# AIflowerQ/InvPref_KDD_2022

Measured on AMD Instinct MI355X. Metric: training interactions/sec, Yahoo-implicit InvPref, higher is better.
Workload: dtype f32; 1 GPU; yahoo_r3_implicit_shaped; users=15400, items=1000, envs=4, factor_num=64, scaling=strong, interactions_total=250154, global_batch=8192, interactions_per_gpu=250154, batch_per_gpu=8192, estep_every_steps=155, parallelism=single GPU

## Files before the change

invpref_kdd_2022_amd/csrc/step_alt.hpp:

```cpp

#ifdef ALT_STAMPS
#define ASTAMP(i) STAMP(i)
#else
#define ASTAMP(i) do { } while (0)
#endif

struct AltArgs {
    float *own_p[2];
    float *own_m[2], *own_v[2];
    const float *oth_p[2];
    float *Ev, *W, *b;
    float *mEv, *mW, *mb, *vEv, *vW, *vb;
    int E, D;
    const int4 *desc;
    const int4 *pend;
    const int4 *list;
    const int *push_slot;
    const int4 *stream;
    int rounds_per_task, rows_per_stream_task, n_cls;
    int cls[8][4];
    const int64_t *envs;
    const float *weights;
    StepScalars k;
    float r2_prev, r1_prev;
    uint32_t flags;
    int mode;
    AdamScalars ad_cur, ad_prev;
    int gen;
    int *sched_state;
    int sched_slot;
    const SchedRow *sched_table;
    int sched_n;
    const float *pend_rows;
    float *push_rows;
    const float *slabs_prev;
    int n_partials_prev;
    float *slabs;
    int *fold_flags;
    unsigned long long *pub;
    float l2, l1;
    double inv_B_prev, inv_BD2_prev;
    float *losses_prev;
    int fold_blocks, first_task_block;
    int stamps_nodrain;
    unsigned long long *stamps;
};

__device__ __forceinline__ float ld_sc1(const float *p) {
    return __hip_atomic_load(p, __ATOMIC_RELAXED, __HIP_MEMORY_SCOPE_AGENT);
}
__device__ __forceinline__ int ld_sc1(const int *p) {
    return __hip_atomic_load(p, __ATOMIC_RELAXED, __HIP_MEMORY_SCOPE_AGENT);
}
__device__ __forceinline__ void st_sc1(float *p, float v) {
    __hip_atomic_store(p, v, __ATOMIC_RELAXED, __HIP_MEMORY_SCOPE_AGENT);
}
__device__ __forceinline__ void st_sc1(int *p, int v) {
    __hip_atomic_store(p, v, __ATOMIC_RELAXED, __HIP_MEMORY_SCOPE_AGENT);
}

#ifndef ALT_POLL_MAX
#define ALT_POLL_MAX (1 << 17)
#endif
#ifndef ALT_TEST_BAD_TAG
#define ALT_TEST_BAD_TAG 0
#endif
constexpr int kAltStreamDelay = 40;
constexpr int kAltPushSt = 1, kAltSlabSt = 1;
constexpr int kAltPendBatch = 4;

struct AltStage {
    unsigned long long g[9];
    float cw;
};
__device__ __forceinline__ void alt_stage_lanes(const AltArgs &a, int lane, bool (&on)[4], bool &onb) {
    constexpr int DP = 64;
#pragma unroll
    for (int i = 0; i < 4; i++) {
        const int idx = lane + 64 * i, e = idx / DP, d = idx - e * DP;
        on[i] = e < a.E && d < a.D;
    }
    onb = lane < a.E;
}
#define ALT_GRANULE_LOADS                                                                                                     \
    "global_load_dwordx2 %0, %9, %11 sc1\n\t"                                                                              \
    "global_load_dwordx2 %1, %9, %11 offset:512 sc1\n\t"                                                                   \
    "global_load_dwordx2 %2, %9, %11 offset:1024 sc1\n\t"                                                                  \
    "global_load_dwordx2 %3, %9, %11 offset:1536 sc1\n\t"                                                                  \
    "global_load_dwordx2 %4, %9, %11 offset:2048 sc1\n\t"                                                                  \
    "global_load_dwordx2 %5, %9, %11 offset:2560 sc1\n\t"                                                                  \
    "global_load_dwordx2 %6, %9, %11 offset:3072 sc1\n\t"                                                                  \
    "global_load_dwordx2 %7, %9, %11 offset:3584 sc1\n\t"                                                                  \
    "global_load_dwordx2 %8, %10, %11 sc1"
__device__ __forceinline__ void alt_stage_issue(const AltArgs &a, AltStage &x) {
    constexpr int EDP = 4 * 64;
    const int lane = threadIdx.x & 63;
    const unsigned o0 = (unsigned)lane * 8u, ob = (unsigned)(2 * EDP + (lane < a.E ? lane : 0)) * 8u;
    asm volatile(ALT_GRANULE_LOADS
                 : "=&v"(x.g[0]), "=&v"(x.g[1]), "=&v"(x.g[2]), "=&v"(x.g[3]), "=&v"(x.g[4]), "=&v"(x.g[5]), "=&v"(x.g[6]),
                   "=&v"(x.g[7]), "=&v"(x.g[8])
                 : "v"(o0), "v"(ob), "s"(a.pub)
                 : "memory");
    x.cw = ((a.flags & INVPREF_WEIGHTS_BY_ENV) && lane < a.E) ? a.weights[lane] : 1.f;
}
__device__ __forceinline__ void alt_stage_finish(const AltArgs &a, AltStage &x, int gen, float *sEv, float *sW, float *sb, float *scw) {
    constexpr int EMAX = 4, EDP = 4 * 64;
    const int lane = threadIdx.x & 63;
    bool on[4], onb;
    alt_stage_lanes(a, lane, on, onb);
    if (ALT_TEST_BAD_TAG) gen ^= 0x40000000;
    const unsigned o0 = (unsigned)lane * 8u, ob = (unsigned)(2 * EDP + (onb ? lane : 0)) * 8u;
    asm volatile("s_waitcnt vmcnt(0)"
                 : "+v"(x.g[0]), "+v"(x.g[1]), "+v"(x.g[2]), "+v"(x.g[3]), "+v"(x.g[4]), "+v"(x.g[5]), "+v"(x.g[6]), "+v"(x.g[7]),
                   "+v"(x.g[8])
                 :
                 : "memory");
    int polls = 0;
    bool timed_out = false;
    for (;;) {
        bool ok = !onb || (int)(x.g[8] >> 32) == gen;
#pragma unroll
        for (int i = 0; i < 4; i++)
// ... 6 lines not shown
        }
        __builtin_amdgcn_s_sleep(4);
        asm volatile(ALT_GRANULE_LOADS "\n\ts_waitcnt vmcnt(0)"
                     : "=&v"(x.g[0]), "=&v"(x.g[1]), "=&v"(x.g[2]), "=&v"(x.g[3]), "=&v"(x.g[4]), "=&v"(x.g[5]), "=&v"(x.g[6]),
                       "=&v"(x.g[7]), "=&v"(x.g[8])
                     : "v"(o0), "v"(ob), "s"(a.pub)
                     : "memory");
    }
    if (timed_out) {
#pragma unroll
        for (int i = 0; i < 9; i++) x.g[i] = 0x7fc00000ull;
    }
#pragma unroll
    for (int i = 0; i < 4; i++) {
        sEv[lane + 64 * i] = on[i] ? __builtin_bit_cast(float, (unsigned)x.g[i]) : 0.f;
        sW[lane + 64 * i] = on[i] ? __builtin_bit_cast(float, (unsigned)x.g[4 + i]) : 0.f;
    }
    if (lane < EMAX) sb[lane] = onb ? __builtin_bit_cast(float, (unsigned)x.g[8]) : 0.f;
    if (lane < EMAX) scw[lane] = x.cw;
}
__device__ __forceinline__ void alt_stage_plain(const AltArgs &a, float *sEv, float *sW, float *sb, float *scw, bool pure) {
    constexpr int EMAX = 4, DP = 64;
    const int lane = threadIdx.x & 63;
    bool on[4], onb;
    alt_stage_lanes(a, lane, on, onb);
#pragma unroll
    for (int i = 0; i < 4; i++) {
        const int idx = lane + 64 * i, e = idx / DP, d = idx - e * DP;
        const bool o = on[i] && !pure;
        sEv[idx] = o ? a.Ev[e * a.D + d] : 0.f;
        sW[idx] = o ? a.W[e * a.D + d] : 0.f;
    }
    if (lane < EMAX) sb[lane] = (onb && !pure) ? a.b[lane] : 0.f;
    if (lane < EMAX) scw[lane] = ((a.flags & INVPREF_WEIGHTS_BY_ENV) && onb && !pure) ? a.weights[lane] : 1.f;
}

template <int THREADS>
struct AltGeo {
    static constexpr int NG = THREADS / 16, WAVES = THREADS / 64, DP = 64, EMAX = 4;
    static constexpr int SLAB = 2 * EMAX * DP + EMAX + kLossSlots;
    static constexpr int sEv = 0, sW = sEv + EMAX * DP, sb = sW + EMAX * DP;
    static constexpr int scw = sb + EMAX;
    static constexpr int mv = scw + EMAX;
    static constexpr int red = mv + WAVES * 4 * 64 * 4;
    static constexpr int total = red + NG * SLAB;
};

__device__ __forceinline__ void adam4_prev(float4 &p, float4 g, float4 &m, float4 &v, const AdamScalars &ad, float2 prev2) {
    AdamScalars ap = ad;
    ap.step_size = prev2.x; ap.bc2_sqrt = prev2.y;
    adam4(p, g, m, v, ap);
}

template <bool VEC, bool FULL, int MODE, int THREADS>
__device__ __forceinline__ void alt_task(const AltArgs &a, int r0, int slab_index, float *lds,
                                         const AdamScalars &ad_cur, float2 prev2, const StepScalars &k, int gen) {
    constexpr int LG = 16, EMAX = 4, UE = 2;
    using G = AltGeo<THREADS>;
    using L = AltGeo<THREADS>;
    static_assert(EvalLds<16, 4>::total == AltGeo<256>::total, "alt_task: the smallest-instance layout");
    constexpr int NG = G::NG, DP = G::DP;
    float *sEv = lds + L::sEv, *sW = lds + L::sW, *sb = lds + L::sb, *scw = lds + L::scw;
    float4 *mv = reinterpret_cast<float4 *>(lds + L::mv);
    float *red = lds + L::red;
    const int lg = threadIdx.x & (LG - 1), grp = threadIdx.x / LG, wave = threadIdx.x >> 6, lane = threadIdx.x & 63;
    float4 *mv_wave = mv + wave * 4 * 64;
    const bool implicit = a.flags & INVPREF_IMPLICIT;
    const bool rw_rec = a.flags & INVPREF_REWEIGHT_REC, rw_cls = a.flags & INVPREF_REWEIGHT_CLS;
    const bool by_env = a.flags & INVPREF_WEIGHTS_BY_ENV;
    const bool reg_env = a.flags & INVPREF_REG_ENV_EMBED;
    const bool pure = a.flags & INVPREF_PURE_MF;
    const bool dense = (a.flags & INVPREF_DENSE_REG) && !(a.flags & INVPREF_REG_ONLY_EMBED) && !pure;
    constexpr bool has_prev = MODE & 1, has_cur = MODE & 2;
    const int D = a.D;
    float *own0 = a.own_p[0], *own1 = a.own_p[1];
    const float *oth0 = a.oth_p[0], *oth1 = a.oth_p[1];

    ASTAMP(0);
    int4 d = a.desc[(r0 * NG + grp) * 2], d1 = a.desc[(r0 * NG + grp) * 2 + 1];
    int4 pd = make_int4(0, 0, 0, 0);
    if (has_prev) pd = a.pend[r0 * NG + grp];
    ASTAMP(1);
    float accLi = 0.f, accLe = 0.f, accLc = 0.f, accL2 = 0.f, accL1 = 0.f;
    float *slab = a.slabs + (int64_t)slab_index * G::SLAB;
    auto slot_of = [&](int g) {
        constexpr int GW = 64 / LG;
        return lds + L::mv + (g / GW) * (4 * 64 * 4) + (g % GW) * 2 * DP;
    };

    {
        constexpr int nr = 1;
        const int r = r0;
        const int4 dd = d, dd1 = d1;
        const int4 pdd = pd;
        const int row = dd.x, meta = dd.y;
        const bool active = row >= 0, leader = meta & 1;
        const int slices_f = (meta >> 1) & 31, mode = (meta >> 6) & 7;
        const int slices = slices_f ? slices_f : 32;
        const bool rpend = has_prev && (meta < 0);
        const int cnt_i = (meta >> 9) & 0x3fffff;
        const int nsmp = (active && has_cur) ? (mode == 7 ? dd.w - dd.z : mode) : 0;
        if (r == r0 + STAMP_ROUND) ASTAMP(2);
        const int s_lo = dd.z, s_hi1 = max(dd.w - 1, dd.z);
        const int *dwords = reinterpret_cast<const int *>(a.desc + (r * NG + grp) * 2);
        auto sample_at = [&](int sidx) {
            USample sm;
            if (FULL) {
                const int *src = mode == 7 ? reinterpret_cast<const int *>(a.list + min(s_lo + sidx, s_hi1)) : dwords + 2 + 3 * min(sidx, 1);
                sm.oth = src[0]; sm.ps = src[1]; sm.y = __builtin_bit_cast(float, src[2]);
            } else if (mode == 7) {
                const int4 q = a.list[dd.z + sidx];
                sm.oth = q.x; sm.ps = q.y; sm.y = __builtin_bit_cast(float, q.z);
            } else if (sidx == 0) { sm.oth = dd.z; sm.ps = dd.w; sm.y = __builtin_bit_cast(float, dd1.x); }
            else { sm.oth = dd1.y; sm.ps = dd1.z; sm.y = __builtin_bit_cast(float, dd1.w); }
            return sm;
        };
        const int rowc = active ? row : 0;
        float4 oi = row4<VEC, FULL>(own0, rowc, D, lg), oe = f4zero();
        float4 mi = row4<VEC, FULL>(a.own_m[0], rowc, D, lg), vi = row4<VEC, FULL>(a.own_v[0], rowc, D, lg);
        float4 me = f4zero(), ve = f4zero();
        if (!pure) {
            oe = row4<VEC, FULL>(own1, rowc, D, lg);
            me = row4<VEC, FULL>(a.own_m[1], rowc, D, lg); ve = row4<VEC, FULL>(a.own_v[1], rowc, D, lg);
        }
        constexpr int PB = kAltPendBatch;
        static_assert(PB * 2 * 64 * 4 <= 4 * G::SLAB && (4 * G::SLAB) % 4 == 0 && G::red % 4 == 0, "landing block: the wave's four slab rows");
        const int npend = (active && has_prev) ? pdd.y - pdd.x : 0;
        const float *pbase = a.pend_rows + (unsigned)(npend > 0 ? pdd.x : 0) * (unsigned)(2 * DP) + lg * 4;
        float *land = red + wave * 4 * G::SLAB;
        auto pland = [&](int s0) {
#pragma unroll
            for (int j = 0; j < PB; j++) {
                if (s0 + j < npend) {
                    const float *p = pbase + (unsigned)(s0 + j) * (unsigned)(2 * DP);
                    __builtin_amdgcn_global_load_lds((const __attribute__((address_space(1))) void *)p,
                                                     (__attribute__((address_space(3))) void *)(land + (2 * j) * 256), 16, 0, 0);
                    if (!pure)
// ... 144 lines not shown
                        gpi = gpe = f4zero();
#pragma nounroll
                        for (int s = 0; s < slices; s++) {
                            f4add(gpi, *reinterpret_cast<const float4 *>(slot_of(lead + s) + lg * 4));
                            f4add(gpe, *reinterpret_cast<const float4 *>(slot_of(lead + s) + DP + lg * 4));
                        }
                    }
                    __syncthreads();
                }
            }
            const float cp = (float)pdd.z;
            if (cp != 0.f) {
                f4fma(gpi, cp, reg_term(oi, a.r2_prev, a.r1_prev));
                f4fma(gpe, cp, reg_term(oe, a.r2_prev, a.r1_prev));
            }
            adam4_prev(oi, gpi, mi, vi, ad_cur, prev2);
            if (!pure) adam4_prev(oe, gpe, me, ve, ad_cur, prev2);
        }
        if (r == r0 + STAMP_ROUND) ASTAMP(3);
        if (!has_cur) {
            if (active && leader) {
                put4<VEC, 0, FULL>(own0, row, D, lg, oi);
                put4<VEC, 0, FULL>(a.own_m[0], row, D, lg, mi);
                put4<VEC, 0, FULL>(a.own_v[0], row, D, lg, vi);
                if (!pure) {
                    put4<VEC, 0, FULL>(own1, row, D, lg, oe);
                    put4<VEC, 0, FULL>(a.own_m[1], row, D, lg, me);
                    put4<VEC, 0, FULL>(a.own_v[1], row, D, lg, ve);
                }
            }
            return;
        }
        mv_wave[0 * 64 + lane] = mi; mv_wave[1 * 64 + lane] = vi;
        if (!pure) { mv_wave[2 * 64 + lane] = me; mv_wave[3 * 64 + lane] = ve; }
        if (r == r0) {
            {
                constexpr int ZR4 = (2 * EMAX * DP + EMAX) / 4;
                static_assert((2 * EMAX * DP + EMAX) % 4 == 0 && G::SLAB % 4 == 0, "16-byte zeroing");
#pragma unroll
                for (int t = 0; t < (4 * ZR4 + 63) / 64; t++) {
                    const int i = lane + 64 * t;
                    if (i < 4 * ZR4) *reinterpret_cast<float4 *>(land + (i / ZR4) * G::SLAB + (i % ZR4) * 4) = f4zero();
                }
            }
            if (wave == 0) {
                if (has_prev && !pure) alt_stage_issue(a, stg);
                if (has_prev && !pure) alt_stage_finish(a, stg, gen, sEv, sW, sb, scw);
                else alt_stage_plain(a, sEv, sW, sb, scw, pure);
            }
            __syncthreads();
            ASTAMP(4);
        }
        float4 gi = f4zero(), ge = f4zero();
        auto step = [&](const Slot &q, bool has) {
            const int e = q.e;
            if (has) {
                const float wq = by_env ? scw[e] : q.w;
                const float w_rec = rw_rec ? wq : 1.f, w_cls = rw_cls ? wq : 1.f;
                const float4 ev = *reinterpret_cast<const float4 *>(sEv + e * DP + lg * 4);
                Eval<EMAX> o;
                eval_interaction<LG, EMAX>(o, oi, q.qi, oe, q.qa, ev, sW, sb, nullptr, a.E, e, q.sm.y, w_rec * k.invB,
                                           w_cls * k.invB, k, implicit, pure, lg);
                float4 gip;
                gip.x = o.g_p - k.alpha * o.gx.x; gip.y = o.g_p - k.alpha * o.gx.y;
                gip.z = o.g_p - k.alpha * o.gx.z; gip.w = o.g_p - k.alpha * o.gx.w;
                f4add(gi, f4mul(gip, q.qi));
                f4fma(ge, o.g_q, f4mul(q.qa, ev));
                float *cr = a.push_rows + (unsigned)q.cs * (unsigned)(2 * DP) + lg * 4;
                store4<kAltPushSt>(cr, f4mul(gip, oi));
                store4<kAltPushSt>(cr + DP, f4scale(o.g_q, f4mul(oe, ev)));
                float4 oo = f4scale(o.g_q, f4mul(oe, q.qa));
                if (reg_env) f4add(oo, reg_term(ev, 2.f * k.r2, 2.f * k.r1));
                float *mine = red + grp * G::SLAB;
#pragma unroll
                for (int c = 0; c < EMAX; c++) {
                    float4 *wr = reinterpret_cast<float4 *>(mine + EMAX * DP + c * DP + lg * 4);
                    float4 cur = *wr;
                    f4fma(cur, o.gz[c], o.x);
                    *wr = cur;
                }
                if (lg == 0) {
                    float4 *br = reinterpret_cast<float4 *>(mine + 2 * EMAX * DP);
                    float4 cur = *br;
                    cur.x += o.gz[0]; cur.y += o.gz[1]; cur.z += o.gz[2]; cur.w += o.gz[3];
                    *br = cur;
                }
                float4 *erow = reinterpret_cast<float4 *>(mine + e * DP + lg * 4);
                float4 cur = *erow;
                f4add(cur, oo);
                *erow = cur;
                float s2a = 0.f, s2b = 0.f;
                sq_acc(s2a, s2b, q.qi);
                sq_acc(s2a, s2b, q.qa);
                float s2 = s2a + s2b, s1 = abs_acc(abs_acc(0.f, q.qi), q.qa);
                if (reg_env) { s2 += 2.f * f4sq(ev); s1 += 2.f * f4abs(ev); }
                accL2 += s2;
                accL1 += s1;
                if (lg == 0) { accLi += o.li * w_rec; accLe += o.le * w_rec; }
                if (lg == 0) accLc += o.lcls * w_cls;
            }
        };
        for (int s = 0; s < nsmp; s += UE) {
#pragma unroll
            for (int j = 0; j < UE; j++) {
                if (s + j < nsmp) step(sl[j], true);
                if (FULL || s + UE + j < nsmp) gather(sl[j], idn[j]);
                if (FULL || s + 2 * UE + j < nsmp) idn[j] = sample_at(s + 2 * UE + j);
            }
        }
        if (r == r0 + STAMP_ROUND) ASTAMP(5);
        const float cnt = (float)cnt_i;
        if (active && leader) {
            accL2 += cnt * (f4sq(oi) + f4sq(oe));
            accL1 += cnt * (f4abs(oi) + f4abs(oe));
        }
        const bool last = r == r0 + nr - 1;
        if (last) {
            accLi = row16_sum(accLi); accLe = row16_sum(accLe); accLc = row16_sum(accLc);
            accL2 = row16_sum(accL2); accL1 = row16_sum(accL1);
            if (lg == 0) {
                float *ls = red + grp * G::SLAB + 2 * EMAX * DP + EMAX;
                ls[0] = accLi; ls[1] = accLe; ls[2] = accLc; ls[3] = accL2; ls[4] = accL1;
                ls[5] = ls[6] = ls[7] = 0.f;
            }
            if (dense && slab_index == 0 && wave == 0) {
                const float4 w4 = *reinterpret_cast<const float4 *>(sW + lane * 4);
                float w2 = f4sq(w4), w1 = f4abs(w4);
                const float bb = lane < EMAX ? sb[lane] : 0.f;
                float b2 = bb * bb, b1 = fabsf(bb);
                w2 = wave_sum_valu(w2); w1 = wave_sum_valu(w1); b2 = wave_sum_valu(b2); b1 = wave_sum_valu(b1);
                if (lane == 0) {
                    float *ls = red + 2 * EMAX * DP + EMAX;
                    ls[5] = w2 / ((float)a.D * (float)a.E) + b2 / (float)a.E;
                    ls[6] = w1 / ((float)a.D * (float)a.E) + b1 / (float)a.E;
                }
            }
        }
        if (active && leader) {
            mi = mv_wave[0 * 64 + lane]; vi = mv_wave[1 * 64 + lane];
            if (!pure) { me = mv_wave[2 * 64 + lane]; ve = mv_wave[3 * 64 + lane]; }
        }
        asm volatile("" ::: "memory");
        if (slices > 1) {
            float *mine = slot_of(grp);
            *reinterpret_cast<float4 *>(mine + lg * 4) = gi;
            *reinterpret_cast<float4 *>(mine + DP + lg * 4) = ge;
        }
        if (slices > 1 || last) __syncthreads();
        if (last) {
            static_assert(G::SLAB % 4 == 0 && G::SLAB / 4 <= THREADS && NG % 8 == 0, "slab sum: one float4 column set per thread");
            if ((int)threadIdx.x < G::SLAB / 4) {
                const float *col = red + threadIdx.x * 4;
                float4 sum = *reinterpret_cast<const float4 *>(col);
#pragma unroll
                for (int q0 = 0; q0 < NG; q0 += 8) {
                    float4 x[8];
#pragma unroll
                    for (int j = 0; j < 8; j++) x[j] = *reinterpret_cast<const float4 *>(col + (q0 + j) * G::SLAB);
#pragma unroll
                    for (int j = (q0 == 0 ? 1 : 0); j < 8; j++) f4add(sum, x[j]);
                }
                store4<kAltSlabSt>(slab + threadIdx.x * 4, sum);
            }
        }
        if (slices > 1) {
            if (active && leader) {
                if (VEC && slices >= 8) {
                    float4 xi[8], xe[8];
#pragma unroll
                    for (int j = 1; j < 8; j++) {
                        xi[j] = *reinterpret_cast<const float4 *>(slot_of(grp + j) + lg * 4);
                        xe[j] = *reinterpret_cast<const float4 *>(slot_of(grp + j) + DP + lg * 4);
                    }
#pragma unroll
                    for (int j = 1; j < 8; j++) { f4add(gi, xi[j]); f4add(ge, xe[j]); }
#pragma nounroll
                    for (int s = 8; s < slices; s += 8) {
#pragma unroll
                        for (int j = 0; j < 8; j++) {
                            xi[j] = *reinterpret_cast<const float4 *>(slot_of(grp + s + j) + lg * 4);
                            xe[j] = *reinterpret_cast<const float4 *>(slot_of(grp + s + j) + DP + lg * 4);
                        }
#pragma unroll
                        for (int j = 0; j < 8; j++) { f4add(gi, xi[j]); f4add(ge, xe[j]); }
                    }
                } else if (VEC && slices == 4) {
                    float4 xi[4], xe[4];
#pragma unroll
                    for (int j = 1; j < 4; j++) {
                        xi[j] = *reinterpret_cast<const float4 *>(slot_of(grp + j) + lg * 4);
                        xe[j] = *reinterpret_cast<const float4 *>(slot_of(grp + j) + DP + lg * 4);
                    }
#pragma unroll
                    for (int j = 1; j < 4; j++) { f4add(gi, xi[j]); f4add(ge, xe[j]); }
                } else {
#pragma nounroll
                    for (int s = 1; s < slices; s++) {
                        f4add(gi, *reinterpret_cast<const float4 *>(slot_of(grp + s) + lg * 4));
                        f4add(ge, *reinterpret_cast<const float4 *>(slot_of(grp + s) + DP + lg * 4));
                    }
                }
            }
            if (!last) __syncthreads();
        }
        if (r == r0 + STAMP_ROUND) ASTAMP(6);
        if (active && leader) {
            if (cnt != 0.f) {
                f4fma(gi, cnt, reg_term(oi, k.r2, k.r1));
                f4fma(ge, cnt, reg_term(oe, k.r2, k.r1));
            }
            adam4(oi, gi, mi, vi, ad_cur);
            put4<VEC, 0, FULL>(own0, row, D, lg, oi);
            put4<VEC, 0, FULL>(a.own_m[0], row, D, lg, mi);
            put4<VEC, 0, FULL>(a.own_v[0], row, D, lg, vi);
            if (!pure) {
// ... 59 lines not shown
#pragma unroll
        for (int q = 0; q < R; q++) {
            float4 gi = f4zero(), ge = f4zero();
            if (has_prev) {
#pragma unroll
                for (int j = 0; j < H; j++) {
                    f4add(gi, j < npend[q] ? ci[q][j] : f4zero());
                    if (!pure) f4add(ge, j < npend[q] ? ce[q][j] : f4zero());
                }
                const float *pb = a.pend_rows + (unsigned)(npend[q] > 0 ? e[q].y : 0) * (unsigned)(2 * DP) + lg * 4;
                for (int s0 = H; s0 < n_wave; s0 += H) {
                    float4 xi[H], xe[H];
#pragma unroll
                    for (int j = 0; j < H; j++) {
                        const int sj = s0 + j < npend[q] ? s0 + j : (npend[q] > 0 ? npend[q] - 1 : 0);
                        xi[j] = *reinterpret_cast<const float4 *>(pb + (unsigned)sj * (unsigned)(2 * DP));
                        xe[j] = pure ? f4zero() : *reinterpret_cast<const float4 *>(pb + (unsigned)sj * (unsigned)(2 * DP) + DP);
                    }
#pragma unroll
                    for (int j = 0; j < H; j++) {
                        f4add(gi, s0 + j < npend[q] ? xi[j] : f4zero());
                        if (!pure) f4add(ge, s0 + j < npend[q] ? xe[j] : f4zero());
                    }
                }
                const float cp = (float)e[q].w;
                if (cp != 0.f) {
                    f4fma(gi, cp, reg_term(p[2 * q], a.r2_prev, a.r1_prev));
                    f4fma(ge, cp, reg_term(p[2 * q + 1], a.r2_prev, a.r1_prev));
                }
                adam4_prev(p[2 * q], gi, m[2 * q], v[2 * q], ad_cur, prev2);
                if (!pure) adam4_prev(p[2 * q + 1], ge, m[2 * q + 1], v[2 * q + 1], ad_cur, prev2);
            }
            if (has_cur) {
                adam4(p[2 * q], f4zero(), m[2 * q], v[2 * q], ad_cur);
                if (!pure) adam4(p[2 * q + 1], f4zero(), m[2 * q + 1], v[2 * q + 1], ad_cur);
            }
            if (on[q]) {
#pragma unroll
                for (int tb = 0; tb < 2; tb++) {
                    if (pure && tb) continue;
                    put4<VEC, kStreamSt, FULL>(a.own_p[tb], e[q].x, D, lg, p[2 * q + tb]);
                    put4<VEC, kStreamSt, FULL>(a.own_m[tb], e[q].x, D, lg, m[2 * q + tb]);
                    put4<VEC, kStreamSt, FULL>(a.own_v[tb], e[q].x, D, lg, v[2 * q + tb]);
                }
            }
        }
    }
}

template <int THREADS>
__device__ __forceinline__ void alt_fold_block(const AltArgs &a, int fb, float *lds, const AdamScalars &ad, int gen) {
    constexpr int kFoldSubs = THREADS / kFoldCols;
    constexpr int DP = 64, EMAX = 4, SLAB = 2 * EMAX * DP + EMAX + kLossSlots, EDP = EMAX * DP;
    double *part = reinterpret_cast<double *>(lds);
    const int colx = threadIdx.x % kFoldCols, sub = threadIdx.x / kFoldCols;
    const int idx = fb * kFoldCols + colx;
    const bool pure = a.flags & INVPREF_PURE_MF;
    const bool dense = (a.flags & INVPREF_DENSE_REG) && !(a.flags & INVPREF_REG_ONLY_EMBED) && !pure;
    const bool mine = idx < SLAB;
    const bool isLoss = idx >= 2 * EDP + EMAX, isB = !isLoss && idx >= 2 * EDP, isW = !isLoss && !isB && idx >= EDP;
    const int rr = isW ? idx - EDP : idx;
    const int e = isB ? idx - 2 * EDP : rr / DP, dd = isB ? 0 : rr - e * DP;
    const bool live = mine && !isLoss && e < a.E && dd < a.D && !pure;
    const int off = live ? (isB ? e : e * a.D + dd) : 0;
    float pre_p = 0.f, pre_m = 0.f, pre_v = 0.f;
    if (sub == 0 && live) {
        pre_p = (isB ? a.b : (isW ? a.W : a.Ev))[off];
        pre_m = (isB ? a.mb : (isW ? a.mW : a.mEv))[off];
        pre_v = (isB ? a.vb : (isW ? a.vW : a.vEv))[off];
    }
    const float *col = a.slabs_prev + (mine ? idx : 0);
    const int np = a.n_partials_prev;
    double acc = 0.0;
    constexpr int CH = kFoldCh;
    for (int s0 = sub; s0 < np; s0 += CH * kFoldSubs) {
        float x[CH];
#pragma unroll
        for (int j = 0; j < CH; j++) x[j] = col[(int64_t)min(s0 + j * kFoldSubs, np - 1) * SLAB];
#pragma unroll
        for (int j = 0; j < CH; j++) acc += (s0 + j * kFoldSubs < np) ? (double)x[j] : 0.0;
    }
    part[sub * kFoldCols + colx] = acc;
    __syncthreads();
    if (sub == 0 && mine) {
        double v = 0.0;
#pragma unroll
        for (int q = 0; q < kFoldSubs; q++) v += part[q * kFoldCols + colx];
        if (!isLoss) {
            if (live) {
                float gv = (float)v, pv = pre_p;
                if (isB) {
                    if (dense) gv += 2.f * a.l2 / (float)a.E * pv + a.l1 / (float)a.E * c_sign(pv);
                } else if (isW && dense) {
                    gv += 2.f * a.l2 / ((float)a.D * (float)a.E) * pv + a.l1 / ((float)a.D * (float)a.E) * c_sign(pv);
                }
                float mm = pre_m, vv = pre_v;
                adam1(pv, gv, mm, vv, ad);
                (isB ? a.b : (isW ? a.W : a.Ev))[off] = pv;
                __hip_atomic_store(a.pub + idx, ((unsigned long long)(unsigned)gen << 32) | (unsigned long long)__builtin_bit_cast(unsigned, pv),
                                   __ATOMIC_RELAXED, __HIP_MEMORY_SCOPE_AGENT);
                (isB ? a.mb : (isW ? a.mW : a.mEv))[off] = mm;
                (isB ? a.vb : (isW ? a.vW : a.vEv))[off] = vv;
            }
        } else {
            double *sl = part + kFoldSubs * kFoldCols;
            sl[idx - 2 * EDP - EMAX] = v;
        }
    }
    __syncthreads();
    constexpr int loss0 = 2 * EDP + EMAX;
    if (fb == loss0 / kFoldCols && threadIdx.x == 0 && a.losses_prev) {
        const double *sl = part + kFoldSubs * kFoldCols;
        const StepScalars &k = a.k;
        const double Li = sl[0] * a.inv_B_prev, Le = sl[1] * a.inv_B_prev, Lc = sl[2] * a.inv_B_prev;
        const double L2 = sl[3] * a.inv_BD2_prev + (dense ? sl[5] : 0.0), L1 = sl[4] * a.inv_BD2_prev + (dense ? sl[6] : 0.0);
        atomicAdd(a.losses_prev + 0, (float)Li); atomicAdd(a.losses_prev + 1, (float)Le); atomicAdd(a.losses_prev + 2, (float)Lc);
        atomicAdd(a.losses_prev + 3, (float)L2); atomicAdd(a.losses_prev + 4, (float)L1);
        atomicAdd(a.losses_prev + 5, (float)((double)k.ca * Li + (double)k.cb * Le + (double)k.cc * Lc + (double)a.l2 * L2 + (double)a.l1 * L1));
    }
}

template <bool VEC, bool FULL, int MODE, int THREADS = 256>
__global__ __launch_bounds__(THREADS, THREADS == 256 ? 3 : 1) void mstep_alt_kernel(AltArgs a) {
    extern __shared__ __attribute__((aligned(16))) float lds[];
    AdamScalars ad_cur = a.ad_cur;
    float2 prev2 = make_float2(a.ad_prev.step_size, a.ad_prev.bc2_sqrt);
    StepScalars k = a.k;
    int gen = a.gen;
    if (a.sched_state) {
        const int *cur = a.sched_state + 16 * a.sched_slot;
        const SchedRow *sr = reinterpret_cast<const SchedRow *>(cur + 2);
        gen = cur[0];
        ad_cur = sr->ad;
        prev2 = (MODE & 2) ? make_float2(__builtin_bit_cast(float, cur[10]), __builtin_bit_cast(float, cur[11]))
                           : make_float2(sr->ad.step_size, sr->ad.bc2_sqrt);
        const float al = sr->alpha;
        if (al == al) k.alpha = al;
    }
    const int b = (int)blockIdx.x;
    if (b < a.first_task_block) {
        if (!(MODE & 1) && b == 0 && threadIdx.x < 63) {
            a.fold_flags[threadIdx.x] = 0;
        }
        if (!(MODE & 1) && b == 0) {
            constexpr int NPUB = 2 * 4 * 64 + 4;
            for (int i = threadIdx.x; i < NPUB; i += THREADS) a.pub[i] = 0ull;
        }
        if (b < a.fold_blocks) {
            if (MODE & 1) {
                ASTAMP(0);
                { AdamScalars adp = ad_cur; adp.step_size = prev2.x; adp.bc2_sqrt = prev2.y; alt_fold_block<THREADS>(a, b, lds, adp, gen); }
                ASTAMP(7);
            }
        } else if (b == a.fold_blocks) {
            if (a.sched_state && (MODE & 2) && threadIdx.x == 0) {
                const int *cur = a.sched_state + 16 * a.sched_slot;
                int *nxt = a.sched_state + 16 * (a.sched_slot ^ 1);
                const int next = cur[0] + 1, base = cur[1], idx = next - base;
                nxt[0] = next;
                nxt[1] = base;
                if (idx >= 0 && idx < a.sched_n) *reinterpret_cast<SchedRow *>(nxt + 2) = a.sched_table[idx];
                nxt[10] = cur[2];
                nxt[11] = cur[3];
            }
        }
        return;
    }
    const int tb = b - a.first_task_block;
    const int ncls = a.n_cls;
    const int c = tb % ncls;
    int j = tb / ncls;
    int q[4] = {0, 0, 0, 0};
#pragma unroll
    for (int kk = 0; kk < 8; kk++) {
        const int on = (c == kk) ? 1 : 0;
#pragma unroll
        for (int i = 0; i < 4; i++) q[i] += a.cls[kk][i] * on;
    }
    const int rpt = a.rounds_per_task, spt = a.rows_per_stream_task;
    const int tj = (q[1] + rpt - 1) / rpt;
    if (j < tj) {
        alt_task<VEC, FULL, MODE, THREADS>(a, q[0] + j, q[0] + j, lds, ad_cur, prev2, k, gen);
        return;
    }
    j -= tj;
    if (j * spt < q[3]) {
        ASTAMP(0);
        if (MODE & 2) stream_delay<kAltStreamDelay>();
        alt_stream<VEC, FULL, MODE, THREADS>(a, a.stream + q[2] + j * spt, min(spt, q[3] - j * spt), ad_cur, prev2);
        ASTAMP(7);
    }
}

inline size_t alt_half_floats(int n_cap, int partials_cap) {
    const size_t rows = ((size_t)(n_cap > 0 ? n_cap : 0) + 1) * 2 * 64;
    const size_t slabs = (size_t)(partials_cap > 0 ? partials_cap : 1) * (2 * 4 * 64 + 4 + kLossSlots);
    return (rows + slabs + 63) & ~(size_t)63;
}
constexpr size_t kAltTailBytes = 64 * sizeof(int) + ((2 * 4 * 64 + 4) * 8 + 255) / 256 * 256;
inline size_t alt_flags_offset(int n_cap, int partials_cap) { return 2 * alt_half_floats(n_cap, partials_cap) * sizeof(float); }

int launch_alt(const InvPrefTables *tables, const InvPrefTables *exp_avg, const InvPrefTables *exp_avg_sq,
               const InvPrefAltPlan *plan, const int64_t *envs, const float *weights, int64_t batch_norm,
               int64_t batch_norm_prev, const InvPrefCoefs *coefs, uint32_t flags, float *losses6_prev, int64_t step, double lr,
               double beta1, double beta2, double eps, const InvPrefAdamSchedule *sched, void *workspace,
               size_t workspace_bytes, int n_cap, int partials_cap, int parity, hipStream_t st) {
    const bool pure = flags & INVPREF_PURE_MF;
    int rc;
    if ((rc = check_tables(tables, pure)) || (rc = check_tables(exp_avg, pure)) || (rc = check_tables(exp_avg_sq, pure))) return rc;
    if (!plan || !coefs || !workspace) return INVPREF_EINVAL;
    if (sched && (!sched->state || !sched->table || sched->n <= 0)) return INVPREF_EINVAL;
    const int D = (int)tables->factor_num, E = (int)tables->env_num;
    if (D > 64 || E > 4) return INVPREF_EUNSUPPORTED;
    const bool has_prev = plan->has_prev != 0, has_cur = plan->has_cur != 0;
    if (!has_prev && !has_cur) return INVPREF_EINVAL;
    if (has_cur && (batch_norm <= 0 || (!envs && !pure) || plan->n <= 0)) return INVPREF_EINVAL;
    if (has_prev && batch_norm_prev <= 0) return INVPREF_EINVAL;
    if (!sched && step < 1) return INVPREF_EINVAL;
    if (pure && (flags & (INVPREF_REWEIGHT_CLS | INVPREF_REG_ENV_EMBED))) return INVPREF_EINVAL;
    if (has_cur && (flags & (INVPREF_REWEIGHT_REC | INVPREF_REWEIGHT_CLS)) && !weights) return INVPREF_EINVAL;
    if ((flags & INVPREF_WEIGHTS_BY_ENV) && pure) return INVPREF_EINVAL;
    if ((uint64_t)(tables->user_num > tables->item_num ? tables->user_num : tables->item_num) * (uint64_t)D * 4ull >= (1ull << 32))
        return INVPREF_EUNSUPPORTED;
    if (plan->lanes_per_group != 16 || (plan->slots_per_round != 16 && plan->slots_per_round != 32) || plan->side < 0 || plan->side > 1 || plan->n < 0 || plan->n_prev < 0 ||
        plan->n_rounds < 0 || plan->rounds_per_task != 1 || plan->n_rounds % plan->rounds_per_task != 0 ||
        plan->n_stream < 0 || plan->rows_per_stream_task <= 0 || (plan->n_rounds > 0 && (!plan->desc || !plan->pend)) ||
        (plan->n > 0 && (!plan->list || !plan->push_slot)) || (plan->n_stream > 0 && !plan->stream) ||
        plan->n > n_cap || plan->n_prev > n_cap || plan->n_partials_prev < 0 || plan->n_partials_prev > partials_cap ||
        (has_cur && plan->n_rounds > partials_cap) || (parity != 0 && parity != 1))
        return INVPREF_EINVAL;
    const int ncls = plan->n_classes > 0 ? plan->n_classes : 1;
    if (ncls > 8) return INVPREF_EINVAL;
    int per_class = 0;
    for (int c = 0; c < ncls; c++) {
        const int32_t *q = plan->cls[c];
        for (int i = 0; i < 4; i++) if (q[i] < 0) return INVPREF_EINVAL;
        if (q[0] + q[1] > plan->n_rounds || q[2] + q[3] > plan->n_stream || q[0] % plan->rounds_per_task) return INVPREF_EINVAL;
        const int tot = (q[1] + plan->rounds_per_task - 1) / plan->rounds_per_task +
                        (q[3] + plan->rows_per_stream_task - 1) / plan->rows_per_stream_task;
        per_class = tot > per_class ? tot : per_class;
    }
    if (workspace_bytes < alt_flags_offset(n_cap, partials_cap) + kAltTailBytes) return INVPREF_EWORKSPACE;
    const size_t half = alt_half_floats(n_cap, partials_cap);
    const size_t rows_floats = ((size_t)n_cap + 1) * 2 * 64;
    float *ws = (float *)workspace;
    AltArgs a{};
    const int s = plan->side;
    float *P[4] = {tables->embed_user_invariant, tables->embed_item_invariant, tables->embed_user_env_aware, tables->embed_item_env_aware};
    float *M[4] = {exp_avg->embed_user_invariant, exp_avg->embed_item_invariant, exp_avg->embed_user_env_aware, exp_avg->embed_item_env_aware};
    float *V[4] = {exp_avg_sq->embed_user_invariant, exp_avg_sq->embed_item_invariant, exp_avg_sq->embed_user_env_aware, exp_avg_sq->embed_item_env_aware};
    for (int tb = 0; tb < 2; tb++) {
        a.own_p[tb] = P[2 * tb + s]; a.own_m[tb] = M[2 * tb + s]; a.own_v[tb] = V[2 * tb + s];
        a.oth_p[tb] = P[2 * tb + (1 - s)];
    }
    a.Ev = tables->embed_env; a.W = tables->classifier_weight; a.b = tables->classifier_bias;
    a.mEv = exp_avg->embed_env; a.mW = exp_avg->classifier_weight; a.mb = exp_avg->classifier_bias;
    a.vEv = exp_avg_sq->embed_env; a.vW = exp_avg_sq->classifier_weight; a.vb = exp_avg_sq->classifier_bias;
    a.E = E; a.D = D;
    a.desc = reinterpret_cast<const int4 *>(plan->desc);
    a.pend = reinterpret_cast<const int4 *>(plan->pend);
    a.list = reinterpret_cast<const int4 *>(plan->list);
    a.push_slot = plan->push_slot;
    a.stream = reinterpret_cast<const int4 *>(plan->stream);
    a.rounds_per_task = plan->rounds_per_task; a.rows_per_stream_task = plan->rows_per_stream_task; a.n_cls = ncls;
    for (int c = 0; c < 8; c++) for (int i = 0; i < 4; i++) a.cls[c][i] = c < ncls ? plan->cls[c][i] : 0;
    a.envs = envs; a.weights = weights;
    a.k = step_scalars(coefs, batch_norm, D);
    if (!has_cur) a.k.invB = a.k.r2 = a.k.r1 = 0.f;
    if (has_prev) {
        a.r2_prev = coefs->L2_coe / ((float)batch_norm_prev * (float)D);
        a.r1_prev = coefs->L1_coe / (2.0f * (float)batch_norm_prev * (float)D);
        a.inv_B_prev = 1.0 / (double)batch_norm_prev;
        a.inv_BD2_prev = 1.0 / ((double)batch_norm_prev * (double)D * 2.0);
    }
    a.flags = flags;
    a.mode = (has_prev ? 1 : 0) | (has_cur ? 2 : 0);
    if (!sched) {
        a.ad_cur = adam_scalars(step, lr, beta1, beta2, eps);
        a.ad_prev = has_cur ? adam_scalars(step > 1 ? step - 1 : 1, lr, beta1, beta2, eps) : a.ad_cur;
        a.gen = (int)step;
    } else {
        a.sched_state = sched->state; a.sched_slot = sched->slot & 1;
        a.sched_table = reinterpret_cast<const SchedRow *>(sched->table); a.sched_n = sched->n;
    }
    float *mine = ws + (size_t)parity * half, *other = ws + (size_t)(1 - parity) * half;
    a.push_rows = mine; a.slabs = mine + rows_floats;
    a.pend_rows = other; a.slabs_prev = other + rows_floats;
    a.n_partials_prev = plan->n_partials_prev;
    a.fold_flags = reinterpret_cast<int *>(reinterpret_cast<char *>(workspace) + alt_flags_offset(n_cap, partials_cap));
    a.pub = reinterpret_cast<unsigned long long *>(reinterpret_cast<char *>(workspace) + alt_flags_offset(n_cap, partials_cap) + 64 * sizeof(int));
    a.l2 = coefs->L2_coe; a.l1 = coefs->L1_coe;
    a.losses_prev = has_prev ? losses6_prev : nullptr;
    constexpr int SLAB = 2 * 4 * 64 + 4 + kLossSlots;
    a.fold_blocks = (SLAB + kFoldCols - 1) / kFoldCols;
    if (a.fold_blocks > 62) return INVPREF_EUNSUPPORTED;
    a.first_task_block = (a.fold_blocks + 1 + 7) & ~7;
    static const char *stamp_env = getenv("INVPREF_STAMPS");
    a.stamps = stamp_env ? reinterpret_cast<unsigned long long *>(strtoull(stamp_env, nullptr, 16)) : nullptr;
    static const bool nodrain = getenv("INVPREF_STAMPS_NODRAIN") != nullptr;
    a.stamps_nodrain = nodrain;
    const int slots = plan->slots_per_round;
    const size_t lds_job = sizeof(float) * (slots == 32 ? AltGeo<512>::total : AltGeo<256>::total);
    const size_t lds_fold = ((size_t)(slots * 16 / kFoldCols) * kFoldCols + kLossSlots) * sizeof(double);
    const size_t lds = lds_job > lds_fold ? lds_job : lds_fold;
    const int grid = a.first_task_block + per_class * ncls;
    const bool vec = vec_ok(tables) && vec_ok(exp_avg) && vec_ok(exp_avg_sq);
    const bool full = vec && D == 64;
    return with_bool(vec, [&](auto vec_c) {
        return with_bool(full, [&](auto full_c) {
            return with_int<256, 512>(slots * 16, [&](auto thr_c) {
                return with_int<1, 2, 3>(a.mode, [&](auto mode_c) {
                    constexpr bool VEC = decltype(vec_c)::value, FULL = decltype(full_c)::value;
                    constexpr int THR = decltype(thr_c)::value;
                    if constexpr (FULL && !VEC) {
                        return (int)INVPREF_EUNSUPPORTED;
                    } else {
                        const auto kernel = mstep_alt_kernel<VEC, FULL, decltype(mode_c)::value, THR>;
                        if ((rc = (int)ensure_lds(kernel, lds))) return rc;
                        hipLaunchKernelGGL(kernel, dim3(grid), dim3(THR), lds, st, a);
                        return (int)hipGetLastError();
                    }
                });
            });
        });
    });
}
```

Before: 527.2 million interactions/s.

## Transpose partial-gradient slabs into per-fold-block column-major layout for coalesced fold reads

Partial-gradient slabs are now stored blocked by fold block, with each fold block's 16 columns contiguous across all partials (stride slab_cap). Fold blocks therefore read contiguous 64-byte chunks per partial instead of strided single floats across whole slabs. The fold loop is also restructured into fixed-capacity chunks with guarded batches of four loads, and the table pointers are chosen once per block. The workspace sizing changes to match, and the producer-side slab stores become scattered across fold-block regions.

```diff
diff --git a/invpref_kdd_2022_amd/csrc/step_alt.hpp b/invpref_kdd_2022_amd/csrc/step_alt.hpp
--- a/invpref_kdd_2022_amd/csrc/step_alt.hpp
+++ b/invpref_kdd_2022_amd/csrc/step_alt.hpp
@@ -35,6 +35,7 @@
     float *push_rows;
     const float *slabs_prev;
     int n_partials_prev;
+    int slab_cap;
     float *slabs;
     int *fold_flags;
     unsigned long long *pub;
@@ -68,6 +69,8 @@
 constexpr int kAltStreamDelay = 40;
 constexpr int kAltPushSt = 1, kAltSlabSt = 1;
 constexpr int kAltPendBatch = 4;
+constexpr int kAltFoldCap = 512;
+constexpr int kAltFoldBlocks = (2 * 4 * 64 + 4 + kLossSlots + kFoldCols - 1) / kFoldCols;
 
 struct AltStage {
     unsigned long long g[9];
@@ -210,7 +213,6 @@
     if (has_prev) pd = a.pend[r0 * NG + grp];
     ASTAMP(1);
     float accLi = 0.f, accLe = 0.f, accLc = 0.f, accL2 = 0.f, accL1 = 0.f;
-    float *slab = a.slabs + (int64_t)slab_index * G::SLAB;
     auto slot_of = [&](int g) {
         constexpr int GW = 64 / LG;
         return lds + L::mv + (g / GW) * (4 * 64 * 4) + (g % GW) * 2 * DP;
@@ -569,7 +571,9 @@
 #pragma unroll
                     for (int j = (q0 == 0 ? 1 : 0); j < 8; j++) f4add(sum, x[j]);
                 }
-                store4<kAltSlabSt>(slab + threadIdx.x * 4, sum);
+                static_assert(kFoldCols == 16, "slab store: four threads' float4 per fold block");
+                float *dst = a.slabs + ((size_t)(threadIdx.x >> 2) * (size_t)a.slab_cap + (size_t)slab_index) * kFoldCols + (threadIdx.x & 3) * 4;
+                store4<kAltSlabSt>(dst, sum);
             }
         }
         if (slices > 1) {
@@ -735,6 +739,8 @@
 __device__ __forceinline__ void alt_fold_block(const AltArgs &a, int fb, float *lds, const AdamScalars &ad, int gen) {
     constexpr int kFoldSubs = THREADS / kFoldCols;
     constexpr int DP = 64, EMAX = 4, SLAB = 2 * EMAX * DP + EMAX + kLossSlots, EDP = EMAX * DP;
+    constexpr int CAP = kAltFoldCap, CH = CAP / kFoldSubs;
+    static_assert(kFoldCols == 16 && CAP % kFoldSubs == 0 && CH % 4 == 0 && EDP % kFoldCols == 0, "fold chunks keep the sub-row classes");
     double *part = reinterpret_cast<double *>(lds);
     const int colx = threadIdx.x % kFoldCols, sub = threadIdx.x / kFoldCols;
     const int idx = fb * kFoldCols + colx;
@@ -746,25 +752,39 @@
     const int e = isB ? idx - 2 * EDP : rr / DP, dd = isB ? 0 : rr - e * DP;
     const bool live = mine && !isLoss && e < a.E && dd < a.D && !pure;
     const int off = live ? (isB ? e : e * a.D + dd) : 0;
+    const int kind = fb < EDP / kFoldCols ? 0 : (fb < 2 * EDP / kFoldCols ? 1 : 2);
+    float *const tab_p = kind == 0 ? a.Ev : (kind == 1 ? a.W : a.b);
+    float *const tab_m = kind == 0 ? a.mEv : (kind == 1 ? a.mW : a.mb);
+    float *const tab_v = kind == 0 ? a.vEv : (kind == 1 ? a.vW : a.vb);
     float pre_p = 0.f, pre_m = 0.f, pre_v = 0.f;
     if (sub == 0 && live) {
-        pre_p = (isB ? a.b : (isW ? a.W : a.Ev))[off];
-        pre_m = (isB ? a.mb : (isW ? a.mW : a.mEv))[off];
-        pre_v = (isB ? a.vb : (isW ? a.vW : a.vEv))[off];
-    }
-    const float *col = a.slabs_prev + (mine ? idx : 0);
+        pre_p = tab_p[off];
+        pre_m = tab_m[off];
+        pre_v = tab_v[off];
+    }
+    const float *colp = a.slabs_prev + (size_t)fb * (size_t)a.slab_cap * kFoldCols + colx;
     const int np = a.n_partials_prev;
     double acc = 0.0;
-    constexpr int CH = kFoldCh;
-    for (int s0 = sub; s0 < np; s0 += CH * kFoldSubs) {
+    for (int c0 = 0; c0 < np; c0 += CAP) {
+        const int n = min(np - c0, CAP);
         float x[CH];
 #pragma unroll
-        for (int j = 0; j < CH; j++) x[j] = col[(int64_t)min(s0 + j * kFoldSubs, np - 1) * SLAB];
-#pragma unroll
-        for (int j = 0; j < CH; j++) acc += (s0 + j * kFoldSubs < np) ? (double)x[j] : 0.0;
-    }
+        for (int j0 = 0; j0 < CH; j0 += 4) {
+            if (j0 * kFoldSubs < n) {
+#pragma unroll
+                for (int j = j0; j < j0 + 4; j++) x[j] = colp[(size_t)(c0 + min(sub + j * kFoldSubs, n - 1)) * kFoldCols];
+            } else {
+#pragma unroll
+                for (int j = j0; j < j0 + 4; j++) x[j] = 0.f;
+            }
+        }
+#pragma unroll
+        for (int j = 0; j < CH; j++) acc += (sub + j * kFoldSubs < n) ? (double)x[j] : 0.0;
+    }
+    ASTAMP(1);
     part[sub * kFoldCols + colx] = acc;
     __syncthreads();
+    ASTAMP(2);
     if (sub == 0 && mine) {
         double v = 0.0;
 #pragma unroll
@@ -779,17 +799,18 @@
                 }
                 float mm = pre_m, vv = pre_v;
                 adam1(pv, gv, mm, vv, ad);
-                (isB ? a.b : (isW ? a.W : a.Ev))[off] = pv;
+                tab_p[off] = pv;
                 __hip_atomic_store(a.pub + idx, ((unsigned long long)(unsigned)gen << 32) | (unsigned long long)__builtin_bit_cast(unsigned, pv),
                                    __ATOMIC_RELAXED, __HIP_MEMORY_SCOPE_AGENT);
-                (isB ? a.mb : (isW ? a.mW : a.mEv))[off] = mm;
-                (isB ? a.vb : (isW ? a.vW : a.vEv))[off] = vv;
+                tab_m[off] = mm;
+                tab_v[off] = vv;
             }
         } else {
             double *sl = part + kFoldSubs * kFoldCols;
             sl[idx - 2 * EDP - EMAX] = v;
         }
     }
+    ASTAMP(3);
     __syncthreads();
     constexpr int loss0 = 2 * EDP + EMAX;
     if (fb == loss0 / kFoldCols && threadIdx.x == 0 && a.losses_prev) {
@@ -877,7 +898,7 @@
 
 inline size_t alt_half_floats(int n_cap, int partials_cap) {
     const size_t rows = ((size_t)(n_cap > 0 ? n_cap : 0) + 1) * 2 * 64;
-    const size_t slabs = (size_t)(partials_cap > 0 ? partials_cap : 1) * (2 * 4 * 64 + 4 + kLossSlots);
+    const size_t slabs = (size_t)(partials_cap > 0 ? partials_cap : 1) * kAltFoldBlocks * kFoldCols;
     return (rows + slabs + 63) & ~(size_t)63;
 }
 constexpr size_t kAltTailBytes = 64 * sizeof(int) + ((2 * 4 * 64 + 4) * 8 + 255) / 256 * 256;
@@ -970,12 +991,12 @@
     a.push_rows = mine; a.slabs = mine + rows_floats;
     a.pend_rows = other; a.slabs_prev = other + rows_floats;
     a.n_partials_prev = plan->n_partials_prev;
+    a.slab_cap = partials_cap > 0 ? partials_cap : 1;
     a.fold_flags = reinterpret_cast<int *>(reinterpret_cast<char *>(workspace) + alt_flags_offset(n_cap, partials_cap));
     a.pub = reinterpret_cast<unsigned long long *>(reinterpret_cast<char *>(workspace) + alt_flags_offset(n_cap, partials_cap) + 64 * sizeof(int));
     a.l2 = coefs->L2_coe; a.l1 = coefs->L1_coe;
     a.losses_prev = has_prev ? losses6_prev : nullptr;
-    constexpr int SLAB = 2 * 4 * 64 + 4 + kLossSlots;
-    a.fold_blocks = (SLAB + kFoldCols - 1) / kFoldCols;
+    a.fold_blocks = kAltFoldBlocks;
     if (a.fold_blocks > 62) return INVPREF_EUNSUPPORTED;
     a.first_task_block = (a.fold_blocks + 1 + 7) & ~7;
     static const char *stamp_env = getenv("INVPREF_STAMPS");
```

After: 527.6 million interactions/s, median of 3. No clear change (+0.1%).

## Evaluate two interactions per group with half-row DPP selection and merged LDS accumulation

Applied to the files above, without the earlier changes.

Replaces the per-sample step with a paired evaluation. Both samples' dot-product reductions run over the full 16-lane group, then the upper and lower eight lanes each take one sample's result, so the sigmoid, BCE and softmax scalar work is done once for two interactions. DPP half-row broadcasts then hand both sets of gradients back to every lane. The classifier weight-gradient slab is read and written once per pair instead of once per sample, and the bias and loss accumulation are merged the same way. This adds DPP shuffles, duplicated reductions and extra control flow (a wave ballot for the odd tail), and any mistake in the lane selection would silently corrupt gradients.

```diff
diff --git a/invpref_kdd_2022_amd/csrc/step_alt.hpp b/invpref_kdd_2022_amd/csrc/step_alt.hpp
--- a/invpref_kdd_2022_amd/csrc/step_alt.hpp
+++ b/invpref_kdd_2022_amd/csrc/step_alt.hpp
@@ -180,6 +180,128 @@
     adam4(p, g, m, v, ap);
 }
 
+template <int BANKS>
+__device__ __forceinline__ float dpp_half(float x) {
+    const int v = __builtin_bit_cast(int, x);
+    return __builtin_bit_cast(float, __builtin_amdgcn_update_dpp(v, v, 0x128, 0xF, BANKS, false));
+}
+template <int EMAX>
+struct EvalPair {
+    float g_p0, g_p1, g_q0, g_q1, gz0[EMAX], gz1[EMAX];
+    float li, le, lcls;
+    float4 x0, x1;
+};
+struct PairSlot {
+    int e;
+    float y, w;
+};
+template <bool TWO, int LG = 16, int EMAX = 4>
+__device__ __forceinline__ void eval_pair(EvalPair<EMAX> &o, float4 pu, float4 pa, float4 qi0, float4 qa0, float4 qi1, float4 qa1,
+                                          PairSlot s0, PairSlot s1, const float *sEv, const float *sW, const float *sb,
+                                          const float *scw, int E, bool by_env, bool rw_rec, bool rw_cls, const StepScalars &k,
+                                          bool implicit, bool pure, int lg) {
+    static_assert(LG == 16 && EMAX == 4, "eval_pair: one DPP row per group, four classes");
+    constexpr int DP = 4 * LG;
+    const bool hi = TWO && (lg & 8);
+    o.x0 = f4mul(pu, qi0);
+    o.x1 = f4zero();
+    float p = group_sum<LG>((o.x0.x + o.x0.y) + (o.x0.z + o.x0.w));
+    float q = group_sum<LG>(dot4(f4mul(pa, qa0), *reinterpret_cast<const float4 *>(sEv + s0.e * DP + lg * 4)));
+    if (TWO) {
+        o.x1 = f4mul(pu, qi1);
+        const float p1 = group_sum<LG>((o.x1.x + o.x1.y) + (o.x1.z + o.x1.w));
+        const float q1 = group_sum<LG>(dot4(f4mul(pa, qa1), *reinterpret_cast<const float4 *>(sEv + s1.e * DP + lg * 4)));
+        p = hi ? p1 : p;
+        q = hi ? q1 : q;
+    }
+    float z[EMAX];
+#pragma unroll
+    for (int c = 0; c < EMAX; c++) z[c] = 0.f;
+    if (!pure) {
+#pragma unroll
+        for (int c = 0; c < EMAX; c++) {
+            const float4 wrow = *reinterpret_cast<const float4 *>(sW + c * DP + lg * 4);
+            z[c] = group_sum<LG>(dot4(o.x0, wrow));
+            if (TWO) {
+                const float z1 = group_sum<LG>(dot4(o.x1, wrow));
+                z[c] = hi ? z1 : z[c];
+            }
+        }
+    }
+    const float y = hi ? s1.y : s0.y;
+    const int e = hi ? s1.e : s0.e;
+    const float wq = by_env ? scw[e] : (hi ? s1.w : s0.w);
+    const float w_rec = rw_rec ? wq : 1.f, w_cls = rw_cls ? wq : 1.f;
+    const float cw_rec = w_rec * k.invB, cw_cls = w_cls * k.invB;
+    float g_p, g_q, li, le, lcls = 0.f, gz[EMAX];
+    if (implicit) {
+        const float sp = f_sigmoid(p), sq = f_sigmoid(q), sv = sp * sq;
+        li = f_bce_binary(sp, y);
+        le = f_bce_binary(sv, y);
+        if (__builtin_amdgcn_ballot_w64(!(y == 0.0f || y == 1.0f)) != 0) {
+            li = f_bce(sp, y);
+            le = f_bce(sv, y);
+        }
+        const float d_inv = k.ca * cw_rec * f_dbce(sp, y);
+        const float d_env = k.cb * cw_rec * f_dbce(sv, y);
+        g_p = (d_inv + d_env * sq) * (sp * (1.f - sp));
+        g_q = d_env * sp * (sq * (1.f - sq));
+    } else {
+        const float s2 = p + q;
+        li = (p - y) * (p - y);
+        le = (s2 - y) * (s2 - y);
+        const float d_env = k.cb * cw_rec * 2.f * (s2 - y);
+        g_p = k.ca * cw_rec * 2.f * (p - y) + d_env;
+        g_q = d_env;
+    }
+#pragma unroll
+    for (int c = 0; c < EMAX; c++) gz[c] = 0.f;
+    if (!pure) {
+        float mx = -__builtin_inff();
+#pragma unroll
+        for (int c = 0; c < EMAX; c++) {
+            const float zc = z[c] + sb[c];
+            z[c] = c < E ? zc : -__builtin_inff();
+            mx = z[c] > mx ? z[c] : mx;
+        }
+        float se = 0.f, zr = 0.f;
+#pragma unroll
+        for (int c = 0; c < EMAX; c++) {
+            const float dz = z[c] - mx;
+            zr = (c == e) ? dz : zr;
+            z[c] = f_exp(dz);
+            se += z[c];
+        }
+        const float rse = f_rcp(se);
+        lcls = f_log(se) - zr;
+#pragma unroll
+        for (int c = 0; c < EMAX; c++) gz[c] = c < E ? k.cc * cw_cls * (z[c] * rse - (c == e ? 1.f : 0.f)) : 0.f;
+    }
+    o.li = li * w_rec;
+    o.le = le * w_rec;
+    o.lcls = lcls * w_cls;
+    if (TWO) {
+        o.g_p0 = dpp_half<0xC>(g_p); o.g_p1 = dpp_half<0x3>(g_p);
+        o.g_q0 = dpp_half<0xC>(g_q); o.g_q1 = dpp_half<0x3>(g_q);
+#pragma unroll
+        for (int c = 0; c < EMAX; c++) { o.gz0[c] = dpp_half<0xC>(gz[c]); o.gz1[c] = dpp_half<0x3>(gz[c]); }
+    } else {
+        o.g_p0 = g_p; o.g_q0 = g_q;
+        o.g_p1 = o.g_q1 = 0.f;
+#pragma unroll
+        for (int c = 0; c < EMAX; c++) { o.gz0[c] = gz[c]; o.gz1[c] = 0.f; }
+    }
+}
+template <int LG = 16, int EMAX = 4>
+__device__ __forceinline__ float4 pair_gx(const float (&gz)[EMAX], const float *sW, bool pure, int lg) {
+    float4 gx = f4zero();
+    if (!pure) {
+#pragma unroll
+        for (int c = 0; c < EMAX; c++) f4fma(gx, gz[c], *reinterpret_cast<const float4 *>(sW + c * (4 * LG) + lg * 4));
+    }
+    return gx;
+}
+
 template <bool VEC, bool FULL, int MODE, int THREADS>
 __device__ __forceinline__ void alt_task(const AltArgs &a, int r0, int slab_index, float *lds,
                                          const AdamScalars &ad_cur, float2 prev2, const StepScalars &k, int gen) {
@@ -461,61 +583,78 @@
             ASTAMP(4);
         }
         float4 gi = f4zero(), ge = f4zero();
-        auto step = [&](const Slot &q, bool has) {
-            const int e = q.e;
-            if (has) {
-                const float wq = by_env ? scw[e] : q.w;
-                const float w_rec = rw_rec ? wq : 1.f, w_cls = rw_cls ? wq : 1.f;
-                const float4 ev = *reinterpret_cast<const float4 *>(sEv + e * DP + lg * 4);
-                Eval<EMAX> o;
-                eval_interaction<LG, EMAX>(o, oi, q.qi, oe, q.qa, ev, sW, sb, nullptr, a.E, e, q.sm.y, w_rec * k.invB,
-                                           w_cls * k.invB, k, implicit, pure, lg);
-                float4 gip;
-                gip.x = o.g_p - k.alpha * o.gx.x; gip.y = o.g_p - k.alpha * o.gx.y;
-                gip.z = o.g_p - k.alpha * o.gx.z; gip.w = o.g_p - k.alpha * o.gx.w;
-                f4add(gi, f4mul(gip, q.qi));
-                f4fma(ge, o.g_q, f4mul(q.qa, ev));
-                float *cr = a.push_rows + (unsigned)q.cs * (unsigned)(2 * DP) + lg * 4;
-                store4<kAltPushSt>(cr, f4mul(gip, oi));
-                store4<kAltPushSt>(cr + DP, f4scale(o.g_q, f4mul(oe, ev)));
-                float4 oo = f4scale(o.g_q, f4mul(oe, q.qa));
-                if (reg_env) f4add(oo, reg_term(ev, 2.f * k.r2, 2.f * k.r1));
-                float *mine = red + grp * G::SLAB;
-#pragma unroll
-                for (int c = 0; c < EMAX; c++) {
-                    float4 *wr = reinterpret_cast<float4 *>(mine + EMAX * DP + c * DP + lg * 4);
-                    float4 cur = *wr;
-                    f4fma(cur, o.gz[c], o.x);
-                    *wr = cur;
-                }
-                if (lg == 0) {
-                    float4 *br = reinterpret_cast<float4 *>(mine + 2 * EMAX * DP);
-                    float4 cur = *br;
-                    cur.x += o.gz[0]; cur.y += o.gz[1]; cur.z += o.gz[2]; cur.w += o.gz[3];
-                    *br = cur;
-                }
-                float4 *erow = reinterpret_cast<float4 *>(mine + e * DP + lg * 4);
-                float4 cur = *erow;
-                f4add(cur, oo);
-                *erow = cur;
-                float s2a = 0.f, s2b = 0.f;
-                sq_acc(s2a, s2b, q.qi);
-                sq_acc(s2a, s2b, q.qa);
-                float s2 = s2a + s2b, s1 = abs_acc(abs_acc(0.f, q.qi), q.qa);
-                if (reg_env) { s2 += 2.f * f4sq(ev); s1 += 2.f * f4abs(ev); }
-                accL2 += s2;
-                accL1 += s1;
-                if (lg == 0) { accLi += o.li * w_rec; accLe += o.le * w_rec; }
-                if (lg == 0) accLc += o.lcls * w_cls;
-            }
+        float *mine = red + grp * G::SLAB;
+        auto back = [&](const Slot &q, const float (&gz)[EMAX], float g_p, float g_q) {
+            const float4 ev = *reinterpret_cast<const float4 *>(sEv + q.e * DP + lg * 4);
+            const float4 gx = pair_gx<LG, EMAX>(gz, sW, pure, lg);
+            float4 gip;
+            gip.x = g_p - k.alpha * gx.x; gip.y = g_p - k.alpha * gx.y;
+            gip.z = g_p - k.alpha * gx.z; gip.w = g_p - k.alpha * gx.w;
+            f4add(gi, f4mul(gip, q.qi));
+            f4fma(ge, g_q, f4mul(q.qa, ev));
+            float *cr = a.push_rows + (unsigned)q.cs * (unsigned)(2 * DP) + lg * 4;
+            store4<kAltPushSt>(cr, f4mul(gip, oi));
+            store4<kAltPushSt>(cr + DP, f4scale(g_q, f4mul(oe, ev)));
+            float4 oo = f4scale(g_q, f4mul(oe, q.qa));
+            if (reg_env) f4add(oo, reg_term(ev, 2.f * k.r2, 2.f * k.r1));
+            float4 *erow = reinterpret_cast<float4 *>(mine + q.e * DP + lg * 4);
+            float4 cur = *erow;
+            f4add(cur, oo);
+            *erow = cur;
+            float s2a = 0.f, s2b = 0.f;
+            sq_acc(s2a, s2b, q.qi);
+            sq_acc(s2a, s2b, q.qa);
+            float s2 = s2a + s2b, s1 = abs_acc(abs_acc(0.f, q.qi), q.qa);
+            if (reg_env) { s2 += 2.f * f4sq(ev); s1 += 2.f * f4abs(ev); }
+            accL2 += s2;
+            accL1 += s1;
         };
         for (int s = 0; s < nsmp; s += UE) {
-#pragma unroll
-            for (int j = 0; j < UE; j++) {
-                if (s + j < nsmp) step(sl[j], true);
-                if (FULL || s + UE + j < nsmp) gather(sl[j], idn[j]);
-                if (FULL || s + 2 * UE + j < nsmp) idn[j] = sample_at(s + 2 * UE + j);
-            }
+            const bool has1 = s + 1 < nsmp;
+            const bool two = __builtin_amdgcn_ballot_w64(has1) != 0;
+            EvalPair<EMAX> o;
+            {
+                const PairSlot s0{sl[0].e, sl[0].sm.y, sl[0].w}, s1{sl[1].e, sl[1].sm.y, sl[1].w};
+                if (two)
+                    eval_pair<true, LG, EMAX>(o, oi, oe, sl[0].qi, sl[0].qa, sl[1].qi, sl[1].qa, s0, s1, sEv, sW, sb, scw, a.E,
+                                              by_env, rw_rec, rw_cls, k, implicit, pure, lg);
+                else
+                    eval_pair<false, LG, EMAX>(o, oi, oe, sl[0].qi, sl[0].qa, sl[1].qi, sl[1].qa, s0, s1, sEv, sW, sb, scw, a.E,
+                                               by_env, rw_rec, rw_cls, k, implicit, pure, lg);
+            }
+            {
+                float4 cw[EMAX];
+#pragma unroll
+                for (int c = 0; c < EMAX; c++) cw[c] = *reinterpret_cast<const float4 *>(mine + EMAX * DP + c * DP + lg * 4);
+#pragma unroll
+                for (int c = 0; c < EMAX; c++) f4fma(cw[c], o.gz0[c], o.x0);
+                if (has1) {
+#pragma unroll
+                    for (int c = 0; c < EMAX; c++) f4fma(cw[c], o.gz1[c], o.x1);
+                }
+#pragma unroll
+                for (int c = 0; c < EMAX; c++) *reinterpret_cast<float4 *>(mine + EMAX * DP + c * DP + lg * 4) = cw[c];
+            }
+            back(sl[0], o.gz0, o.g_p0, o.g_q0);
+            if (FULL || s + UE < nsmp) gather(sl[0], idn[0]);
+            if (FULL || s + 2 * UE < nsmp) idn[0] = sample_at(s + 2 * UE);
+            if (has1) back(sl[1], o.gz1, o.g_p1, o.g_q1);
+            const float li1 = dpp_xor<8>(o.li, lg), le1 = dpp_xor<8>(o.le, lg), lc1 = dpp_xor<8>(o.lcls, lg);
+            if (lg == 0) {
+                float4 *br = reinterpret_cast<float4 *>(mine + 2 * EMAX * DP);
+                float4 cur = *br;
+                cur.x += o.gz0[0]; cur.y += o.gz0[1]; cur.z += o.gz0[2]; cur.w += o.gz0[3];
+                accLi += o.li; accLe += o.le;
+                accLc += o.lcls;
+                if (has1) {
+                    cur.x += o.gz1[0]; cur.y += o.gz1[1]; cur.z += o.gz1[2]; cur.w += o.gz1[3];
+                    accLi += li1; accLe += le1;
+                    accLc += lc1;
+                }
+                *br = cur;
+            }
+            if (FULL || s + UE + 1 < nsmp) gather(sl[1], idn[1]);
+            if (FULL || s + 2 * UE + 1 < nsmp) idn[1] = sample_at(s + 2 * UE + 1);
         }
         if (r == r0 + STAMP_ROUND) ASTAMP(5);
         const float cnt = (float)cnt_i;
```

After: 526.2 million interactions/s before, 527.9 million interactions/s after (median of 4 runs). No clear change (+0.3%).
